# bcgsc/ntJoin

Hardware: AMD Instinct MI355X
Metric: Gbp/s minimizer-sketch+graph-build (k=32,w=1000) (higher is better)
Workload: dtype u64

## Files before the change

ntjoin_amd/csrc/graph.hip:

```cpp
#include <algorithm>
#include <cstdlib>
#include <cstring>
#include <system_error>
#include <thread>

#include "join_verdict.h"
#include "mxg_internal.h"
#include "scan_kernels.h"

namespace mxg {

static constexpr uint64_t HT_EMPTY = 0xFFFFFFFFFFFFFFFFull;
static constexpr uint32_t NONE32 = 0xFFFFFFFFu;

struct Slot {
    unsigned long long key;
    uint32_t nseen, ndup;
};

__device__ __forceinline__ uint32_t ht_slot(Slot *tab, uint32_t mask, uint32_t cap, uint64_t key)
{
    if (key == HT_EMPTY) return cap;
    uint32_t s = (uint32_t)((key * 0x9E3779B97F4A7C15ull) >> 32) & mask;
    while (true) {
// ... 158 lines not shown
            const uint32_t cb = hist[b0 + u];
            start[b0 + u] = run;
            row[b0 + u] = run;
            hist[b0 + u] = 0;
            run += cb;
        }
    if (threadIdx.x == 0) row[P] = sh[255];
    __syncthreads();
#pragma unroll
    for (uint32_t u = 0; u < U; ++u) {
        if (!((live >> u) & 1u)) continue;
        const uint32_t blk = blk0 + u * BPU + sub;
        uint32_t a = a0, i = ib0 + (u * BPU + sub) * 256u + t256;
        if (!one) {
            a = asm_of_block(p, blk);
            i = (blk - p.bstart[a]) * 256u + t256;
        }
        const uint32_t b = pj_part(key[u], pmask);
        const uint32_t pos = j * PJ_IPB + start[b] + atomicAdd(&hist[b], 1u);
        recs[pos] = make_uint4((uint32_t)key[u], (uint32_t)(key[u] >> 32), i, a | (((dupm >> u) & 1u) ? PJ_REC_DUP : 0u));
    }
}

__device__ __forceinline__ uint32_t pj_slot(unsigned long long *keys, uint64_t key)
{
    if (key == HT_EMPTY) return PJ_T;
    uint32_t s = (uint32_t)((key * 0x9E3779B97F4A7C15ull) >> 32) & (PJ_T - 1u);
    for (uint32_t step = 0; step < PJ_T; ++step) {
        const unsigned long long cur = keys[s];
        if (cur == key) return s;
        if (cur == HT_EMPTY) {
            const unsigned long long old = atomicCAS(&keys[s], (unsigned long long)HT_EMPTY, (unsigned long long)key);
            if (old == HT_EMPTY || old == key) return s;
        }
        s = (s + 1u) & (PJ_T - 1u);
    }
    return PJ_T + 1u;
}

struct PjSub {
    uint32_t n_sub, s, off, cap;
};
struct PjSubCaps {
    uint32_t n_sub;
    uint32_t cap[MXG_MAX_ASSEMBLIES];
};
template <bool NARROW>
__global__ __launch_bounds__(256) void k_pj_join(uint4 *recs, const uint32_t *__restrict__ M, uint32_t P, uint32_t n_rows,
                                                 uint64_t *host_fail, uint32_t force_fail, const uint32_t *__restrict__ cursor,
                                                 uint32_t cap1, uint32_t rows2, const AsmSet p, const PjSubCaps caps)
{
    const uint32_t full = p.full;
    __shared__ unsigned long long keys[PJ_T + 1];
    __shared__ uint32_t seen[PJ_T + 1], dup[NARROW ? 1 : PJ_T + 1];
    __shared__ uint32_t item0[PJ_T + 1];
    __shared__ uint32_t seg_off[257], seg_rec[256], sh[256];
    __shared__ uint32_t failed;
    uint32_t b = blockIdx.x, rec_off = 0;
    if (cursor) {
        const uint32_t c = blockIdx.x / P;
        b = blockIdx.x % P;
        n_rows = caps.n_sub > 1 ? rows2 : (min(cursor[c * PJ1_CS], cap1) + PJ_IPB - 1) / PJ_IPB;
        M += (size_t)c * rows2 * (P + 1);
        rec_off = c * cap1;
        if (threadIdx.x == 0)
            for (uint32_t s = 0; s < caps.n_sub; ++s)
                if (cursor[(c * caps.n_sub + s) * PJ1_CS] > caps.cap[s]) *host_fail = 1;
    }
    for (uint32_t s = threadIdx.x; s <= PJ_T; s += 256) {
        keys[s] = HT_EMPTY;
        seen[s] = 0;
        if (!NARROW) dup[s] = 0;
    }
// ... 42 lines not shown
                                if (NARROW) atomicOr(&seen[s], bit | (bit << 16));
                                else {
                                    atomicOr(&seen[s], bit);
                                    atomicOr(&dup[s], bit);
                                }
                            } else if (atomicOr(&seen[s], bit) & bit) {
                                if (NARROW) atomicOr(&seen[s], bit << 16); else atomicOr(&dup[s], bit);
                            }
                            if (last_a == 0) item0[s] = rec.z;
                        }
                    }
                }
                return s;
            };
            auto insert = [&](uint32_t r) { return insert_rec(recs[r]); };
            auto finish = [&](uint32_t i, uint32_t s, uint32_t a) {
                uint32_t fl = 0;
                if (!bad) {
                    const uint32_t sn = seen[s] & full, d = (NARROW ? seen[s] >> 16 : dup[s]) & full;
                    const bool inall = sn == full;
                    fl = (!(d & (1u << a)) ? MXG_MX_UNIQUE : 0u) | ((inall && d == 0) ? MXG_MX_SHARED : 0u) | (inall ? MXG_MX_INALL : 0u);
                }
                const uint32_t word = ((fl & MXG_MX_SHARED) ? item0[s] << 3 : 0u) | fl;
                if (!pj_verdict_is_prefill(word)) p.slot[a][i] = word;
            };
#pragma unroll
            for (uint32_t it = 0; it < QC; ++it) {
                const uint32_t q = threadIdx.x + it * 256u;
                if (q >= total) break;
                if (pass == 0) {
                    rc[it] = locate(q);
                    sc[it] = insert(rc[it]);
                    ac[it] = last_a;
                    ic[it] = last_i;
                } else if (single) {
                    finish(ic[it], sc[it], ac[it]);
                } else {
                    const uint32_t r = locate(q);
                    const uint32_t s = insert(r);
                    finish(last_i, s, last_a);
                }
            }
            constexpr uint32_t TU = 8;
            for (uint32_t q0 = threadIdx.x + QC * 256u; q0 < total; q0 += 256u * TU) {
                uint4 rv[TU];
#pragma unroll
                for (uint32_t u = 0; u < TU; ++u) {
                    const uint32_t q = q0 + u * 256u;
                    rv[u] = q < total ? recs[locate(q)] : make_uint4(0u, 0u, 0u, 0u);
                }
#pragma unroll
                for (uint32_t u = 0; u < TU; ++u) {
                    if (q0 + u * 256u >= total) break;
                    const uint32_t s = insert_rec(rv[u]);
                    if (pass == 1) finish(last_i, s, last_a);
                }
            }
            __syncthreads();
        }
    }
}


template <bool NARROW>
__global__ __launch_bounds__(256) void k_pj_join_pipe(uint4 *recs, const uint32_t *__restrict__ M, uint32_t P, uint32_t n_parts,
                                                      uint64_t *host_fail, uint32_t force_fail, const uint32_t *__restrict__ cursor,
                                                      uint32_t cap1, uint32_t rows2, const AsmSet p, const PjSubCaps caps)
{
    const uint32_t full = p.full;
    __shared__ unsigned long long keys[PJ_T + 1];
    __shared__ uint32_t seen[PJ_T + 1], dup[NARROW ? 1 : PJ_T + 1];
    __shared__ uint32_t item0[PJ_T + 1];
    __shared__ uint32_t seg_off[2][257], seg_rec[2][256], sh[256];
    __shared__ uint32_t failed;
    constexpr uint32_t QC = 4;
    __shared__ uint8_t seg_of[QC * 256];
    uint4 rn[QC];
    uint32_t tot_n = 0;
    uint32_t lo_nn = 0, len_nn = 0;
    auto bounds = [&](uint32_t part, uint32_t &lo, uint32_t &len) {
        lo = len = 0;
        if (part < n_parts && threadIdx.x < rows2) {
            const uint32_t c = part / P, b = part % P;
            const uint32_t *row = M + ((size_t)c * rows2 + threadIdx.x) * (P + 1);
            lo = row[b];
            len = row[b + 1];
        }
    };
    auto lay_out = [&](uint32_t part, uint32_t buf, uint32_t lo, uint32_t end) {
        const uint32_t c = part < n_parts ? part / P : 0u;
        const uint32_t len = end - lo;
        const uint32_t off = block_exclusive_256(len, sh);
        seg_off[buf][threadIdx.x] = off;
        seg_rec[buf][threadIdx.x] = c * cap1 + threadIdx.x * PJ_IPB + lo;
        for (uint32_t q = off, e = min(off + len, QC * 256u); q < e; ++q) seg_of[q] = (uint8_t)threadIdx.x;
        const uint32_t total = sh[255];
        __syncthreads();
#pragma unroll
        for (uint32_t it = 0; it < QC; ++it) {
            const uint32_t q = threadIdx.x + it * 256u;
            rn[it] = make_uint4(0u, 0u, 0u, 0u);
            if (q < total) {
                const uint32_t l = seg_of[q];
                rn[it] = recs[seg_rec[buf][l] + (q - seg_off[buf][l])];
            }
        }
        return total;
    };
    const uint32_t first = blockIdx.x, stride = gridDim.x;
    {
        uint32_t lo, end;
        bounds(first, lo, end);
        bounds(first + stride, lo_nn, len_nn);
        tot_n = lay_out(first, 0u, lo, end);
    }
    uint32_t k = 0;
    for (uint32_t part = first; part < n_parts; part += stride, ++k) {
        uint4 rc[QC];
#pragma unroll
        for (uint32_t it = 0; it < QC; ++it) rc[it] = rn[it];
        const uint32_t total = tot_n, buf = k & 1u;
        {
            const uint32_t lo = lo_nn, end = len_nn;
            bounds(part + 2u * stride, lo_nn, len_nn);
            tot_n = lay_out(part + stride, buf ^ 1u, lo, end);
        }
        for (uint32_t s = threadIdx.x; s <= PJ_T; s += 256) {
            keys[s] = HT_EMPTY;
            seen[s] = 0;
            if (!NARROW) dup[s] = 0;
        }
        if (threadIdx.x == 0) {
            failed = force_fail;
            const uint32_t c = part / P;
            if (part % P == 0)
                for (uint32_t s = 0; s < caps.n_sub; ++s)
                    if (cursor[(c * caps.n_sub + s) * PJ1_CS] > caps.cap[s]) *host_fail = 1;
        }
        __syncthreads();
        auto locate = [&](uint32_t q) {
            uint32_t l = 0, h = 256;
            while (h - l > 1) {
                const uint32_t m = (l + h) >> 1;
                if (seg_off[buf][m] <= q) l = m; else h = m;
            }
            return seg_rec[buf][l] + (q - seg_off[buf][l]);
        };
        auto insert_rec = [&](const uint4 rec, bool record) {
            const uint32_t a = rec.w & ~PJ_REC_DUP;
            const uint32_t s = pj_slot(keys, ((uint64_t)rec.y << 32) | rec.x);
            if (record) {
                const uint32_t bit = 1u << a;
                if (s > PJ_T) failed = 1;
                else {
                    const uint32_t cur = seen[s], dcur = NARROW ? cur >> 16 : dup[s];
                    if (!((cur & bit) && (dcur & bit))) {
                        if (rec.w & PJ_REC_DUP) {
                            if (NARROW) atomicOr(&seen[s], bit | (bit << 16));
                            else {
                                atomicOr(&seen[s], bit);
                                atomicOr(&dup[s], bit);
                            }
                        } else if (atomicOr(&seen[s], bit) & bit) {
                            if (NARROW) atomicOr(&seen[s], bit << 16); else atomicOr(&dup[s], bit);
                        }
                        if (a == 0) item0[s] = rec.z;
                    }
                }
            }
            return s;
        };
        uint32_t sc[QC];
#pragma unroll
        for (uint32_t it = 0; it < QC; ++it)
            if (threadIdx.x + it * 256u < total) sc[it] = insert_rec(rc[it], true);
        constexpr uint32_t TU = 8;
        for (uint32_t q0 = threadIdx.x + QC * 256u; q0 < total; q0 += 256u * TU) {
            uint4 rv[TU];
#pragma unroll
            for (uint32_t u = 0; u < TU; ++u) {
                const uint32_t q = q0 + u * 256u;
                rv[u] = q < total ? recs[locate(q)] : make_uint4(0u, 0u, 0u, 0u);
            }
#pragma unroll
            for (uint32_t u = 0; u < TU; ++u)
                if (q0 + u * 256u < total) insert_rec(rv[u], true);
        }
        __syncthreads();
        const bool bad = failed != 0;
        if (bad && threadIdx.x == 0) *host_fail = 1;
        auto finish = [&](const uint4 rec, uint32_t s) {
            const uint32_t a = rec.w & ~PJ_REC_DUP;
            uint32_t fl = 0;
            if (!bad) {
                const uint32_t sn = seen[s] & full, d = (NARROW ? seen[s] >> 16 : dup[s]) & full;
                const bool inall = sn == full;
                fl = (!(d & (1u << a)) ? MXG_MX_UNIQUE : 0u) | ((inall && d == 0) ? MXG_MX_SHARED : 0u) | (inall ? MXG_MX_INALL : 0u);
            }
            const uint32_t word = ((fl & MXG_MX_SHARED) ? item0[s] << 3 : 0u) | fl;
            if (!pj_verdict_is_prefill(word)) p.slot[a][rec.z] = word;
        };
#pragma unroll
        for (uint32_t it = 0; it < QC; ++it)
            if (threadIdx.x + it * 256u < total) finish(rc[it], bad ? 0u : sc[it]);
        for (uint32_t q0 = threadIdx.x + QC * 256u; q0 < total; q0 += 256u * TU) {
            uint4 rv[TU];
#pragma unroll
            for (uint32_t u = 0; u < TU; ++u) {
                const uint32_t q = q0 + u * 256u;
                rv[u] = q < total ? recs[locate(q)] : make_uint4(0u, 0u, 0u, 0u);
            }
#pragma unroll
            for (uint32_t u = 0; u < TU; ++u)
                if (q0 + u * 256u < total) finish(rv[u], bad ? 0u : insert_rec(rv[u], false));
        }
        __syncthreads();
    }
}

__device__ __forceinline__ uint32_t pj1_part(uint64_t key, uint32_t p1mask) { return (uint32_t)((key * 0x9E3779B97F4A7C15ull) >> 52) & p1mask; }

__global__ __launch_bounds__(PJ_BT) void k_pj1_scatter(const AsmSet p, uint32_t blk_lo, uint32_t blk_hi, uint32_t p1mask, uint32_t cap1,
                                                     uint32_t *cursor, uint4 *recs1, uint32_t *sup, uint32_t n_sup, const PjSub subr)
{
    extern __shared__ uint32_t pj_lds[];
    uint32_t *hist = pj_lds, *start = pj_lds + p1mask + 1;
    if (blockIdx.x == 0)
        for (uint32_t i = threadIdx.x; i < n_sup; i += PJ_BT) sup[i] = 0;
    constexpr uint32_t U = PJ_IPB / PJ_BT, BPU = PJ_BT / 256;
    const uint32_t j = blockIdx.x, sub = threadIdx.x >> 8, t256 = threadIdx.x & 255u;
    const uint32_t blk0 = blk_lo + j * (PJ_IPB / 256);
    uint64_t key[U];
    uint32_t ia[U], ii[U], live = 0;
#pragma unroll
    for (uint32_t u = 0; u < U; ++u) {
        const uint32_t blk = blk0 + u * BPU + sub;
        key[u] = 0;
        ia[u] = ii[u] = 0;
        if (blk >= blk_hi) continue;
        const uint32_t a = subr.n_sub > 1 ? subr.s : asm_of_block(p, blk);
        const uint32_t i = (blk - p.bstart[a]) * 256u + t256, n = asm_n(p, a);
        const bool lv = i < n;
        if (lv) {
            key[u] = p.hash[a][i];
            p.slot[a][i] = PJ_VERDICT_PREFILL;
        }
        const uint32_t role = pj_run_role(i, n, key[u], lv);
        const uint64_t fb = __ballot(role & 1u);
        if ((threadIdx.x & 63u) == 0) p.fol[(size_t)blk * 4u + ((threadIdx.x >> 6) & 3u)] = fb;
        if (lv && !(role & 1u)) {
            ia[u] = a | ((role & 2u) ? PJ_REC_DUP : 0u);
            ii[u] = i;
            live |= 1u << u;
        }
    }
    for (uint32_t b = threadIdx.x; b <= p1mask; b += PJ_BT) hist[b] = 0;
    __syncthreads();
#pragma unroll
    for (uint32_t u = 0; u < U; ++u)
        if ((live >> u) & 1u) atomicAdd(&hist[pj1_part(key[u], p1mask)], 1u);
    __syncthreads();
    for (uint32_t b = threadIdx.x; b <= p1mask; b += PJ_BT) {
        const uint32_t c = hist[b];
        start[b] = c ? atomicAdd(&cursor[(b * subr.n_sub + subr.s) * PJ1_CS], c) : 0u;
        hist[b] = 0;
    }
    __syncthreads();
#pragma unroll
    for (uint32_t u = 0; u < U; ++u) {
        if (!((live >> u) & 1u)) continue;
        const uint32_t b = pj1_part(key[u], p1mask);
        const uint32_t pos = start[b] + atomicAdd(&hist[b], 1u);
        if (pos < subr.cap) recs1[(size_t)b * cap1 + subr.off + pos] = make_uint4((uint32_t)key[u], (uint32_t)(key[u] >> 32), ii[u], ia[u]);
        else p.slot[ia[u] & ~PJ_REC_DUP][ii[u]] = 0;
    }
}

__global__ __launch_bounds__(PJ_BT) void k_pj2_bucket(const AsmSet p, const uint4 *__restrict__ recs1, const uint32_t *__restrict__ cursor,
                                                    uint32_t cap1, uint32_t rows2, uint32_t pmask, uint32_t *M, uint4 *recs2,
                                                    uint32_t skew_lim, const PjSub subr)
{
    extern __shared__ uint32_t pj_lds[];
    uint32_t *hist = pj_lds, *start = pj_lds + pmask + 1;
    __shared__ uint32_t sh[256];
    const uint32_t j = blockIdx.x, c = blockIdx.y;
    const uint32_t n_all = cursor[(c * subr.n_sub + subr.s) * PJ1_CS], n_c = min(n_all, subr.cap);
    const uint32_t row_j = subr.off / PJ_IPB + j;
    if (j * PJ_IPB >= n_c) {
        uint32_t *row = M + ((size_t)c * rows2 + row_j) * (pmask + 2);
        for (uint32_t b = threadIdx.x; b <= pmask + 1; b += PJ_BT) row[b] = 0;
        return;
    }
    constexpr uint32_t U = PJ_IPB / PJ_BT;
    const size_t base = (size_t)c * cap1 + subr.off + (size_t)j * PJ_IPB;
    uint4 rec[U];
    uint32_t live = 0;
#pragma unroll
    for (uint32_t u = 0; u < U; ++u) {
        const uint32_t q = u * PJ_BT + threadIdx.x;
        rec[u] = make_uint4(0u, 0u, 0u, 0u);
        if (j * PJ_IPB + q < n_c) {
            rec[u] = recs1[base + q];
            live |= 1u << u;
        }
    }
    if (n_all > skew_lim) {
        __shared__ unsigned long long skey[PJ_IPB];
        __shared__ uint32_t sitem[PJ_IPB];
        __shared__ uint8_t sasm[PJ_IPB];
        __shared__ uint32_t stab[PJ_IPB];
        __shared__ uint32_t sdup[PJ_IPB / 32];
        for (uint32_t q = threadIdx.x; q < PJ_IPB; q += PJ_BT) stab[q] = 0xFFFFFFFFu;
        for (uint32_t q = threadIdx.x; q < PJ_IPB / 32; q += PJ_BT) sdup[q] = 0;
#pragma unroll
        for (uint32_t u = 0; u < U; ++u) {
            const uint32_t q = u * PJ_BT + threadIdx.x;
            skey[q] = ((unsigned long long)rec[u].y << 32) | rec[u].x;
            sitem[q] = rec[u].z;
            sasm[q] = (uint8_t)(rec[u].w & 0xFFu);
        }
        __syncthreads();
#pragma unroll
        for (uint32_t u = 0; u < U; ++u) {
            if (!((live >> u) & 1u)) continue;
            const uint32_t q = u * PJ_BT + threadIdx.x;
// ... 12 lines not shown
                if (skey[cur] == key && sasm[cur] == a) {
                    rep = cur;
                    break;
                }
                hsl = (hsl + 1u) & (2u * PJ_IPB - 1u);
            }
            if (rep != q) {
                atomicOr(&sdup[rep >> 5], 1u << (rep & 31u));
                p.slot[a][rec[u].z] = (sitem[rep] << 3) | PJ_VERDICT_REF;
                live &= ~(1u << u);
            }
        }
        __syncthreads();
#pragma unroll
        for (uint32_t u = 0; u < U; ++u) {
            const uint32_t q = u * PJ_BT + threadIdx.x;
            if ((sdup[q >> 5] >> (q & 31u)) & 1u) rec[u].w |= PJ_REC_DUP;
        }
    }
    for (uint32_t b = threadIdx.x; b <= pmask; b += PJ_BT) hist[b] = 0;
    __syncthreads();
#pragma unroll
    for (uint32_t u = 0; u < U; ++u)
        if ((live >> u) & 1u) atomicAdd(&hist[pj_part(((uint64_t)rec[u].y << 32) | rec[u].x, pmask)], 1u);
    __syncthreads();
    const uint32_t P = pmask + 1, per = P >= PJ_BT ? P / PJ_BT : 1u, b0 = threadIdx.x * per;
    uint32_t cn = 0;
    if (b0 < P)
        for (uint32_t u = 0; u < per; ++u) cn += hist[b0 + u];
    uint32_t run = block_exclusive<PJ_BT / 64>(cn, sh);
    uint32_t *row = M + ((size_t)c * rows2 + row_j) * (P + 1);
    if (b0 < P)
        for (uint32_t u = 0; u < per; ++u) {
            const uint32_t cb = hist[b0 + u];
            start[b0 + u] = run;
            row[b0 + u] = run;
            hist[b0 + u] = 0;
            run += cb;
        }
    if (threadIdx.x == 0) row[P] = sh[255];
    __syncthreads();
#pragma unroll
    for (uint32_t u = 0; u < U; ++u) {
        if (!((live >> u) & 1u)) continue;
        const uint32_t b = pj_part(((uint64_t)rec[u].y << 32) | rec[u].x, pmask);
        const uint32_t pos = (uint32_t)base + start[b] + atomicAdd(&hist[b], 1u);
        recs2[pos] = rec[u];
    }
}

template <uint32_t U>
struct TailScan {
    uint32_t tot[U][4];
    uint32_t before[U];
};
template <uint32_t U>
__device__ __forceinline__ void tail_ballot(TailScan<U> &ts, uint32_t u, bool f, uint64_t &bm)
{
    bm = __ballot(f);
    if ((threadIdx.x & 63u) == 0) ts.tot[u][threadIdx.x >> 6] = (uint32_t)__popcll(bm);
}
template <uint32_t U>
__device__ __forceinline__ uint32_t tail_rank(const TailScan<U> &ts, uint32_t u, uint64_t bm)
{
    const uint32_t lane = threadIdx.x & 63u, wv = threadIdx.x >> 6;
    uint32_t r = (uint32_t)__popcll(bm & ((1ull << lane) - 1ull));
#pragma unroll
    for (uint32_t q = 0; q < 3; ++q) r += q < wv ? ts.tot[u][q] : 0u;
    return r;
}
// ... 501 lines not shown
};

static int plan_join(mxg_handle *h, int mode, const GraphBounds *gb, bool global_table, bool split, JoinPlan &pl)
{
    const uint32_t A = (uint32_t)h->asms.size();
    if (A == 0) return set_err(h, MXG_EINVAL, "mxg_build_graph: no assemblies");
    if (A > MXG_MAX_ASSEMBLIES) return set_err(h, MXG_ELIMIT, "at most %d assemblies", MXG_MAX_ASSEMBLIES);
    pl = JoinPlan();
    JoinRequest rq;
    rq.A = A;
    for (uint32_t ai = 0; ai < A; ++ai) {
        Assembly *a = h->asms[ai];
        if (!gb && !a->has_sketch) return set_err(h, MXG_EINVAL, "assembly '%s' has no sketch (call mxg_sketch)", a->name.c_str());
        rq.n_of[ai] = gb ? gb->n_bound[ai] : a->n_mx;
    }
    rq.mode = mode;
    rq.bounds = gb != nullptr;
    rq.global_table = global_table;
    rq.split = split;
    const char *join_env = knob_raw(h, "MXG_GRAPH_JOIN");
    rq.join_global = join_env && !strcmp(join_env, "global");
    rq.force_two_level = knob_u64(h, "MXG_PJ_TWO_LEVEL", 0) != 0;
    rq.graph_u = (uint32_t)std::min<uint64_t>(knob_u64(h, "MXG_GRAPH_U", 0), 8);
    switch (join_shape(rq, h->pj_learnt, pl)) {
    case JS_TOO_MANY_MINIMIZERS: return set_err(h, MXG_ELIMIT, "too many minimizers for one table (%llu)", (unsigned long long)pl.N);
    case JS_TOO_MANY_ITEMS: return set_err(h, MXG_ELIMIT, "graph too large for 32-bit item indices");
    case JS_OK: break;
    }
    pl.pj_force_fail = knob_u64(h, "MXG_PJ_FORCE_FAIL", 0) ? 1u : 0u;
    pl.sc.n_sub = pl.n_sub;
    for (uint32_t a = 0; a < MXG_MAX_ASSEMBLIES; ++a) pl.sc.cap[a] = pl.sub_cap[a];
    const uint64_t *const n_of = pl.n_of;
    const uint32_t nb = pl.nb, P = pl.P, P1 = pl.P1;

    if (!pl.pj) MXG_HIP(h, h->g_keys.ensure(((size_t)pl.cap + 1) * sizeof(Slot)));
    const size_t nb0 = pl.nb0, nb_all = nb;
    MXG_HIP(h, h->g_vid.ensure(pl.pj ? (nb0 + nb_all) * 4 * 8 + nb0 * 4 + 64 : ((size_t)pl.cap + 1) * 4));
    pl.pj_mask0 = h->g_vid.as<uint64_t>();
    uint64_t *const pj_fol = pl.pj_mask0 + nb0 * 4;
    pl.pj_bpref0 = reinterpret_cast<uint32_t *>(pj_fol + nb_all * 4);
    MXG_HIP(h, h->g_ctl.ensure(CTL_WORDS * 8));

    AsmSet &as_all = pl.as_all;
    as_all.n_asm = A;
    as_all.full = pl.full;
    as_all.fol = pl.pj ? pj_fol : nullptr;
// ... 27 lines not shown
        const size_t n_recs = (size_t)P1 * pl.cap1;
        MXG_HIP(h, h->g_part.ensure((size_t)P1 * pl.rows2 * (P + 1) * 4 + (size_t)P1 * PJ1_CS * 4));
        MXG_HIP(h, h->g_keys.ensure(n_recs * sizeof(uint4)));
        MXG_HIP(h, h->g_recs1.ensure(n_recs * sizeof(uint4)));
        pl.M = h->g_part.as<uint32_t>();
        pl.cursor = pl.n_cur ? pl.esup + pl.n_esup : pl.M + (size_t)P1 * pl.rows2 * (P + 1);
        pl.recs1 = h->g_recs1.as<uint4>();
        pl.recs2 = h->g_keys.as<uint4>();
    }
    return MXG_OK;
}

static void launch_partition(mxg_handle *h, const JoinPlan &pl, uint32_t a_lo, uint32_t a_hi, hipStream_t st, uint32_t n_sup_clear)
{
    const uint32_t blk_lo = pl.as_all.bstart[a_lo], blk_hi = pl.as_all.bstart[a_hi];
    const uint32_t n_rows1 = (blk_hi - blk_lo + PJ_IPB / 256 - 1) / (PJ_IPB / 256);
    PjSub sub{1u, 0u, 0u, pl.cap1};
    uint32_t skew_lim = (uint32_t)std::min<uint64_t>(pl.N / pl.P1 + pl.N / pl.P1 / 32 + 2048, 0xFFFFFFFFull);
    if (pl.split) {
        sub = PjSub{pl.A, a_lo, pl.sub_off[a_lo], pl.sub_cap[a_lo]};
        skew_lim = pl.skew_lim[a_lo];
    }
    if (n_rows1)
        hipLaunchKernelGGL(k_pj1_scatter, dim3(n_rows1), dim3(PJ_BT), (size_t)pl.P1 * 8, st, pl.as_all, blk_lo, blk_hi, pl.P1 - 1, pl.cap1,
                           pl.cursor, pl.recs1, pl.fsup, n_sup_clear, sub);
    hipLaunchKernelGGL(k_pj2_bucket, dim3(sub.cap / PJ_IPB, pl.P1), dim3(PJ_BT), (size_t)pl.P * 8, st, pl.as_all, pl.recs1, pl.cursor, pl.cap1,
                       pl.rows2, pl.P - 1, pl.M, pl.recs2, knob_u64(h, "MXG_PJ_SKEW", 0) ? 0u : skew_lim, sub);
}

static int ev_pair(mxg_handle *h, hipEvent_t *a, hipEvent_t *b)
{
    while (h->ev_pool.size() < h->ev_used + 2) {
        hipEvent_t e;
        MXG_HIP(h, hipEventCreate(&e));
        h->ev_pool.push_back(e);
    }
    *a = h->ev_pool[h->ev_used];
    *b = h->ev_pool[h->ev_used + 1];
    h->ev_used += 2;
    h->ev_spans.push_back(TimedSpan{*a, *b, 0, false, 5});
    return MXG_OK;
}

int graph_plan_early(mxg_handle *h, const GraphBounds &gb, bool *early)
{
    *early = false;
    h->pj_early_done = 0;
    if (knob_u64(h, "MXG_PJ_EARLY", 1) == 0) return MXG_OK;
    MXG_HIP(h, hipSetDevice(h->device));
    if (!h->pj_plan) h->pj_plan = new JoinPlan;
// ... 75 lines not shown
          fine((h_->cfg.flags & MXG_FLAG_TIMING_FINE) != 0 && c_.mode == GRAPH_FULL), timing((h_->cfg.flags & MXG_FLAG_TIMING) != 0 || fine),
          g(h_->graph)
    {
    }
    bool joins() const { return pl.nb && !resume; }
    size_t anv() const { return (size_t)pl.A * pl.nvs; }

    int begin()
    {
        for (uint32_t ai = 0; ai < pl.A; ++ai) {
            Assembly *a = h->asms[ai];
            if (!resume) a->flags_on_host = false;
            a->flags_valid = true;
        }
        if (!resume) g = Graph();
        g.n_asm = pl.A;
        if (fine && !h->ev_g[0]) {
            MXG_HIP(h, hipEventCreate(&h->ev_g[0]));
            MXG_HIP(h, hipEventCreate(&h->ev_g[1]));
        }
        if (timing) MXG_HIP(h, hipEventRecord(h->ev0, h->stream));
        if (!resume)
            h->stat_graph_join = (pl.pj ? (pl.two_level ? MXG_JOIN_LDS_TWO_LEVEL : MXG_JOIN_LDS) : MXG_JOIN_GLOBAL) | (early ? MXG_JOIN_EARLY : 0);
        if (!pl.pj && !resume) MXG_HIP(h, hipMemsetAsync(h->g_keys.p, 0xFF, ((size_t)pl.cap + 1) * sizeof(Slot), h->stream));
        ctl = h->g_ctl.as<uint64_t>();
        if (!h->pinned_gctl) MXG_HIP(h, hipHostMalloc((void **)&h->pinned_gctl, CTL_WORDS * 8));
        hctl = h->pinned_gctl;
        memset(hctl, 0, CTL_WORDS * 8);
        pj_fail = pl.dg_pj ? dg_pj_fail_word(h) : hctl + CTL_PJ_FAIL;
        return MXG_OK;
    }

    void launch_join(uint4 *recs, uint32_t *M, uint32_t n_parts, uint32_t n_rows, const uint32_t *cursor)
    {
        const bool narrow = pl.A <= 16;
        const uint32_t cap1 = cursor ? pl.cap1 : 0u, rows2 = cursor ? pl.rows2 : 0u;
        const uint64_t pipe_blocks = cursor ? knob_u64(h, "MXG_PJ_PIPE", 1024) : 0;
        if (pipe_blocks && rows2 <= 256)
            hipLaunchKernelGGL(narrow ? k_pj_join_pipe<true> : k_pj_join_pipe<false>, dim3((uint32_t)std::min<uint64_t>(pipe_blocks, n_parts)),
                               dim3(256), 0, h->stream, recs, M, pl.P, n_parts, pj_fail, pl.pj_force_fail, cursor, cap1, rows2, pl.as_all, pl.sc);
        else
            hipLaunchKernelGGL(narrow ? k_pj_join<true> : k_pj_join<false>, dim3(n_parts), dim3(256), 0, h->stream, recs, M, pl.P, n_rows,
                               pj_fail, pl.pj_force_fail, cursor, cap1, rows2, pl.as_all, pl.sc);
    }
    void flags_pj()
    {
        TAIL_LAUNCH(k_flags_pj, pl.u_flags, dim3(graph_tail_grid(pl.nb, pl.u_flags)), h->stream, pl.as_all, pl.nb, pl.cnt, pl.fsup, pl.pj_mask0);
    }
    int join_two_level()
    {
        if (!early) {
            MXG_HIP(h, hipMemsetAsync(pl.cursor, 0, (size_t)pl.P1 * PJ1_CS * 4, h->stream));
            launch_partition(h, pl, 0, pl.A, h->stream, pl.n_fsup + pl.n_esup);
        }
        launch_join(pl.recs2, pl.M, pl.P1 * pl.P, 0u, pl.cursor);
        flags_pj();
        return MXG_OK;
    }
    int join_one_level()
    {
        const uint32_t n_rows = (pl.nb + PJ_IPB / 256 - 1) / (PJ_IPB / 256);
        MXG_HIP(h, h->g_part.ensure((size_t)n_rows * (pl.P + 1) * 4));
        MXG_HIP(h, h->g_keys.ensure((size_t)n_rows * PJ_IPB * sizeof(uint4)));
        uint32_t *M = h->g_part.as<uint32_t>();
        uint4 *recs = h->g_keys.as<uint4>();
        hipLaunchKernelGGL(k_pj_bucket, dim3(n_rows), dim3(PJ_BT), (size_t)pl.P * 8, h->stream, pl.as_all, pl.nb, pl.P - 1, M, recs, pl.fsup,
                           pl.n_fsup + pl.n_esup);
        launch_join(recs, M, pl.P, n_rows, nullptr);
        flags_pj();
        return MXG_OK;
    }
    int join_global()
    {
        hipLaunchKernelGGL(k_insert, dim3(pl.nb), dim3(256), 0, h->stream, pl.as_all, h->g_keys.as<Slot>(), pl.mask, pl.cap, pl.fsup,
// ... 151 lines not shown
        TAIL_LAUNCH(k_edges, pl.u_edges, grid, h->stream, ep, n_items);
        MXG_HIP(h, hipGetLastError());
        return MXG_OK;
    }

    int sync_and_verdict()
    {
        if (timing) MXG_HIP(h, hipEventRecord(h->ev1, h->stream));
        MXG_HIP(h, stream_wait(h->stream));
        if (!pl.pj || !hctl[CTL_PJ_FAIL]) return MXG_OK;
        if (!pl.two_level || pl.pj_force_fail) return RC_RETRY_GLOBAL;
        std::vector<uint32_t> cur((size_t)pl.P1 * pl.n_sub * PJ1_CS);
        MXG_HIP(h, hipMemcpy(cur.data(), pl.cursor, cur.size() * 4, hipMemcpyDeviceToHost));
        return join_overflow_verdict(pl, cur.data(), h->pj_learnt);
    }
    int results()
    {
        const uint64_t nv = hctl[CTL_SHARED];
        for (uint32_t a = 1; a < pl.A; ++a)
            if (hctl[CTL_SHARED + a] != nv)
                return set_err(h, MXG_EDEVICE, "internal error: shared-minimizer counts differ between assemblies (%llu vs %llu)",
                               (unsigned long long)hctl[CTL_SHARED + a], (unsigned long long)nv);
        g.nv = nv;
        g.nv_stride = pl.nvs;
        g.ne = pl.nvs > 0 ? hctl[CTL_EDGES] : 0;
        h->stat_unique = ~0ull;
        if (timing) {
            float ms = 0;
            MXG_HIP(h, hipEventElapsedTime(&ms, h->ev0, h->ev1));
            h->tm.ms_graph += ms;
            if (fine && pl.nvs > 0) {
                float a = 0, b = 0, c3 = 0;
                MXG_HIP(h, hipEventElapsedTime(&a, h->ev0, h->ev_g[0]));
                MXG_HIP(h, hipEventElapsedTime(&b, h->ev_g[0], h->ev_g[1]));
                MXG_HIP(h, hipEventElapsedTime(&c3, h->ev_g[1], h->ev1));
                h->tm.ms_join += a;
                h->tm.ms_vertices += b;
                h->tm.ms_edges += c3;
            }
        }
        g.valid = true;
        g.own_order = c.mode == GRAPH_FULL;
        g.host_valid = false;
        return MXG_OK;
    }
};
// ... 88 lines not shown
```

ntjoin_amd/csrc/join_plan.h:

```cpp
#pragma once
#include <algorithm>
#include <cstddef>
#include <cstdint>

#include "ntjoin_mx.h"

namespace mxg {

enum { GRAPH_FULL = 0, GRAPH_DG_VERTICES = 1, GRAPH_DG_EDGES = 2, GRAPH_DG_EDGES_APPLIED = 3  };

constexpr uint32_t PJ_IPB = 4096;
constexpr uint32_t PJ_T = 2048;
constexpr uint32_t PJ_MAX_P = 4096;
constexpr uint32_t PJ1_CS = 32;
constexpr uint32_t PJ_CAP_LIMIT = 0xFFFFF000u;

struct JoinLearnt {
    bool overflowed = false;
    uint32_t cap1_P1 = 0;
    uint64_t cap1_need = 0;
    uint64_t sig = 0;
    uint32_t sub_P1 = 0;
    uint64_t sub_need[MXG_MAX_ASSEMBLIES] = {};
    bool dg_off = false;

    static uint64_t signature(uint32_t n_asm, const uint64_t *n_mx)
    {
        uint64_t s = 0x9E3779B97F4A7C15ull * ((uint64_t)n_asm + 1);
        for (uint32_t a = 0; a < n_asm; ++a) s = (s ^ n_mx[a]) * 0x100000001B3ull;
        return s;
    }
    void sketches_are(uint64_t s)
    {
        if ((overflowed || cap1_P1) && sig != s) {
            overflowed = false;
            cap1_P1 = 0;
            cap1_need = 0;
            sub_P1 = 0;
        }
        sig = s;
    }
    void assembly_added()
    {
        overflowed = false;
        cap1_P1 = 0;
        cap1_need = 0;
    }
    void gave_up() { overflowed = true; }
};

struct JoinRequest {
    uint32_t A = 0;
    uint64_t n_of[MXG_MAX_ASSEMBLIES] = {};
    int mode = GRAPH_FULL;
    bool bounds = false;
    bool global_table = false;
    bool split = false;
    bool force_two_level = false;
    bool join_global = false;
    uint32_t graph_u = 0;
};

enum JoinShapeError { JS_OK = 0, JS_TOO_MANY_MINIMIZERS, JS_TOO_MANY_ITEMS };

struct JoinShape {
    uint32_t A = 0;
    uint64_t N = 0, nvs = 0;
    uint64_t n_of[MXG_MAX_ASSEMBLIES] = {};
    uint32_t cap = 0, mask = 0, full = 0;
    uint32_t P = 0, P1 = 0, cap1 = 0, rows2 = 0;
    bool two_level = false, pj = false, dg_pj = false;
    bool split = false;
    uint32_t n_sub = 1;
    uint32_t sub_cap[MXG_MAX_ASSEMBLIES] = {}, sub_off[MXG_MAX_ASSEMBLIES] = {}, skew_lim[MXG_MAX_ASSEMBLIES] = {};
    uint32_t bstart[MXG_MAX_ASSEMBLIES + 1] = {};
    uint32_t nb = 0;
    size_t nb0 = 0;
    uint32_t n_items = 0, e_blocks = 0;
    size_t n_cur = 0;
    uint32_t u_flags = 1, u_vertices = 1, u_edges = 1;
};

constexpr uint32_t GRAPH_TAIL_U2 = 3072, GRAPH_TAIL_U4 = 8192;
constexpr uint32_t GRAPH_TAIL_U_VERTICES = 2;
inline uint32_t graph_tail_u(uint64_t blocks, uint32_t forced = 0)
{
    if (forced == 1 || forced == 2 || forced == 4) return forced;
    return blocks >= GRAPH_TAIL_U4 ? 4u : blocks >= GRAPH_TAIL_U2 ? 2u : 1u;
}
inline uint32_t graph_tail_grid(uint64_t blocks, uint32_t U) { return (uint32_t)((blocks + U - 1) / U); }

inline JoinShapeError join_shape(const JoinRequest &rq, const JoinLearnt &learnt, JoinShape &pl)
{
    pl = JoinShape();
    const uint32_t A = pl.A = rq.A;
    uint64_t N = 0, nmin = ~0ull, n_max = 0;
    for (uint32_t a = 0; a < A; ++a) {
        pl.n_of[a] = rq.n_of[a];
        N += rq.n_of[a];
        nmin = std::min(nmin, rq.n_of[a]);
        n_max = std::max(n_max, rq.n_of[a]);
// ... 34 lines not shown
            cap1 = (uint32_t)((c1 + PJ_IPB - 1) / PJ_IPB * PJ_IPB);
            pl.sub_cap[0] = cap1;
        }
        pl.rows2 = cap1 / PJ_IPB;
    }
    pl.P = P;
    pl.P1 = P1;
    pl.cap1 = cap1;
    pl.two_level = P1 != 0 && P1 <= 4096 && fits32 && (uint64_t)P1 * cap1 < (1ull << 32) && (uint64_t)P1 * P * (PJ_T + 1) < (1ull << 29);
    pl.dg_pj = rq.mode == GRAPH_DG_VERTICES && rq.bounds && !learnt.dg_off;
    pl.pj = (rq.mode == GRAPH_FULL || pl.dg_pj) && !rq.global_table && (P1 == 0 || pl.two_level) && P <= PJ_MAX_P && n_max < (1ull << 29) &&
            !rq.join_global;
    for (uint32_t a = 0; a < A; ++a) {
        pl.bstart[a] = pl.nb;
        pl.nb += (uint32_t)((rq.n_of[a] + 255) / 256);
    }
    for (uint32_t a = A; a <= MXG_MAX_ASSEMBLIES; ++a) pl.bstart[a] = pl.nb;
    pl.nb0 = (size_t)((rq.n_of[0] + 255) / 256);
    pl.nvs = nmin;
    if (pl.nvs > 0 && (uint64_t)A * pl.nvs >= (1ull << 32)) return JS_TOO_MANY_ITEMS;
    pl.n_items = (uint32_t)((size_t)A * pl.nvs);
    pl.e_blocks = (pl.n_items + 255) / 256;
    if (pl.split && pl.pj && pl.two_level) pl.n_cur = (size_t)P1 * A * PJ1_CS;
    pl.u_flags = graph_tail_u(pl.nb, rq.graph_u);
    pl.u_vertices = graph_tail_u(0, rq.graph_u) == rq.graph_u ? rq.graph_u : std::min(pl.u_flags, GRAPH_TAIL_U_VERTICES);
    pl.u_edges = graph_tail_u(pl.e_blocks, rq.graph_u);
    return JS_OK;
}

enum JoinRetry { RC_RETRY_GLOBAL = 1, RC_RETRY_PJ = 2 };

inline JoinRetry join_overflow_verdict(const JoinShape &pl, const uint32_t *cur, JoinLearnt &learnt)
{
    const uint32_t P1 = pl.P1, n_sub = pl.n_sub;
    uint64_t mx = 0;
    for (uint32_t c = 0; c < P1; ++c) {
        uint64_t all = 0;
        for (uint32_t s = 0; s < n_sub; ++s) all += cur[((size_t)c * n_sub + s) * PJ1_CS];
        mx = std::max(mx, all);
    }
    if (pl.split) {
        bool grew = false;
        if (learnt.sub_P1 != P1) std::fill_n(learnt.sub_need, MXG_MAX_ASSEMBLIES, 0ull);
        learnt.sub_P1 = P1;
        for (uint32_t s = 0; s < n_sub; ++s) {
            uint64_t ms = 0;
// ... 22 lines not shown
```

ntjoin_amd/csrc/join_verdict.h:

```cpp
#pragma once
#include <cstdint>

#include "ntjoin_mx.h"

#if defined(__HIPCC__)
#define PJV_HD __host__ __device__ inline
#else
#define PJV_HD inline
#endif

namespace mxg {

constexpr uint32_t PJ_VERDICT_PREFILL = MXG_MX_UNIQUE;
constexpr uint32_t PJ_VERDICT_REF = 2u;

PJV_HD bool pj_verdict_is_prefill(uint32_t word) { return word == PJ_VERDICT_PREFILL; }

}
```

Measured before the change: 2709.

## Pack join records to 12 bytes and learn a shared-prefill verdict

Join records shrink from 16 to 12 bytes. The assembly tag and dup flag are folded into key bits that the partition index already implies, and keys are pre-multiplied so the partition and slot come straight from the stored bits. A learnt prefill rule writes the likely shared verdict for assembly 0 up front so fewer verdict stores are needed on later runs. It also adds a split-per-assembly partition path and debug knobs, which makes the bit-packing and learnt state more complex and adds correctness risk.

```diff
diff --git a/ntjoin_amd/csrc/graph.hip b/ntjoin_amd/csrc/graph.hip
--- a/ntjoin_amd/csrc/graph.hip
+++ b/ntjoin_amd/csrc/graph.hip
@@ -204,10 +204,9 @@
     }
 }
 
-__device__ __forceinline__ uint32_t pj_slot(unsigned long long *keys, uint64_t key)
+__device__ __forceinline__ uint32_t pj_slot_from(unsigned long long *keys, uint64_t key, uint32_t s)
 {
     if (key == HT_EMPTY) return PJ_T;
-    uint32_t s = (uint32_t)((key * 0x9E3779B97F4A7C15ull) >> 32) & (PJ_T - 1u);
     for (uint32_t step = 0; step < PJ_T; ++step) {
         const unsigned long long cur = keys[s];
         if (cur == key) return s;
@@ -218,6 +217,27 @@
         s = (s + 1u) & (PJ_T - 1u);
     }
     return PJ_T + 1u;
+}
+__device__ __forceinline__ uint32_t pj_slot(unsigned long long *keys, uint64_t key)
+{
+    return pj_slot_from(keys, key, (uint32_t)((key * 0x9E3779B97F4A7C15ull) >> 32) & (PJ_T - 1u));
+}
+
+struct PjRec3 {
+    uint32_t x, y, z;
+};
+template <bool R12>
+__device__ __forceinline__ uint4 pj_rec_load(const uint4 *recs, size_t r)
+{
+    if (!R12) return recs[r];
+    const PjRec3 v = reinterpret_cast<const PjRec3 *>(recs)[r];
+    return make_uint4(v.x, v.y, v.z, 0u);
+}
+template <bool R12>
+__device__ __forceinline__ void pj_rec_store(uint4 *recs, size_t r, const uint4 v)
+{
+    if (!R12) recs[r] = v;
+    else reinterpret_cast<PjRec3 *>(recs)[r] = PjRec3{v.x, v.y, v.z};
 }
 
 struct PjSub {
@@ -230,7 +250,7 @@
 template <bool NARROW>
 __global__ __launch_bounds__(256) void k_pj_join(uint4 *recs, const uint32_t *__restrict__ M, uint32_t P, uint32_t n_rows,
                                                  uint64_t *host_fail, uint32_t force_fail, const uint32_t *__restrict__ cursor,
-                                                 uint32_t cap1, uint32_t rows2, const AsmSet p, const PjSubCaps caps)
+                                                 uint32_t cap1, uint32_t rows2, const AsmSet p, const PjSubCaps caps, uint32_t prefill0)
 {
     const uint32_t full = p.full;
     __shared__ unsigned long long keys[PJ_T + 1];
@@ -319,7 +339,7 @@
                     fl = (!(d & (1u << a)) ? MXG_MX_UNIQUE : 0u) | ((inall && d == 0) ? MXG_MX_SHARED : 0u) | (inall ? MXG_MX_INALL : 0u);
                 }
                 const uint32_t word = ((fl & MXG_MX_SHARED) ? item0[s] << 3 : 0u) | fl;
-                if (!pj_verdict_is_prefill(word)) p.slot[a][i] = word;
+                if (word != pj_verdict_prefill(prefill0, a, i)) p.slot[a][i] = word;
             };
 #pragma unroll
             for (uint32_t it = 0; it < QC; ++it) {
@@ -359,12 +379,19 @@
 }
 
 
-template <bool NARROW>
+template <bool NARROW, bool R12>
 __global__ __launch_bounds__(256) void k_pj_join_pipe(uint4 *recs, const uint32_t *__restrict__ M, uint32_t P, uint32_t n_parts,
                                                       uint64_t *host_fail, uint32_t force_fail, const uint32_t *__restrict__ cursor,
-                                                      uint32_t cap1, uint32_t rows2, const AsmSet p, const PjSubCaps caps)
+                                                      uint32_t cap1, uint32_t rows2, const AsmSet p, const PjSubCaps caps, uint32_t prefill0)
 {
     const uint32_t full = p.full;
+    const uint32_t lgP = R12 ? 31u - (uint32_t)__clz(P) : 0u, tag_mask = R12 ? pj12_tag_mask(lgP) : 0u;
+    auto rec_a = [&](const uint4 rec) { return R12 ? pj12_unpack_tag(rec.y, lgP) & (PJ12_TAG_DUP - 1u) : rec.w & ~PJ_REC_DUP; };
+    auto rec_dup = [&](const uint4 rec) { return R12 ? (pj12_unpack_tag(rec.y, lgP) & PJ12_TAG_DUP) != 0 : (rec.w & PJ_REC_DUP) != 0; };
+    auto rec_slot = [&](unsigned long long *tab, const uint4 rec) {
+        if (R12) return pj_slot_from(tab, ((uint64_t)(rec.y & ~tag_mask) << 32) | rec.x, rec.y & (PJ_T - 1u));
+        return pj_slot(tab, ((uint64_t)rec.y << 32) | rec.x);
+    };
     __shared__ unsigned long long keys[PJ_T + 1];
     __shared__ uint32_t seen[PJ_T + 1], dup[NARROW ? 1 : PJ_T + 1];
     __shared__ uint32_t item0[PJ_T + 1];
@@ -399,7 +426,7 @@
             rn[it] = make_uint4(0u, 0u, 0u, 0u);
             if (q < total) {
                 const uint32_t l = seg_of[q];
-                rn[it] = recs[seg_rec[buf][l] + (q - seg_off[buf][l])];
+                rn[it] = pj_rec_load<R12>(recs, seg_rec[buf][l] + (q - seg_off[buf][l]));
             }
         }
         return total;
@@ -444,15 +471,15 @@
             return seg_rec[buf][l] + (q - seg_off[buf][l]);
         };
         auto insert_rec = [&](const uint4 rec, bool record) {
-            const uint32_t a = rec.w & ~PJ_REC_DUP;
-            const uint32_t s = pj_slot(keys, ((uint64_t)rec.y << 32) | rec.x);
+            const uint32_t a = rec_a(rec);
+            const uint32_t s = rec_slot(keys, rec);
             if (record) {
                 const uint32_t bit = 1u << a;
                 if (s > PJ_T) failed = 1;
                 else {
                     const uint32_t cur = seen[s], dcur = NARROW ? cur >> 16 : dup[s];
                     if (!((cur & bit) && (dcur & bit))) {
-                        if (rec.w & PJ_REC_DUP) {
+                        if (rec_dup(rec)) {
                             if (NARROW) atomicOr(&seen[s], bit | (bit << 16));
                             else {
                                 atomicOr(&seen[s], bit);
@@ -477,7 +504,7 @@
 #pragma unroll
             for (uint32_t u = 0; u < TU; ++u) {
                 const uint32_t q = q0 + u * 256u;
-                rv[u] = q < total ? recs[locate(q)] : make_uint4(0u, 0u, 0u, 0u);
+                rv[u] = q < total ? pj_rec_load<R12>(recs, locate(q)) : make_uint4(0u, 0u, 0u, 0u);
             }
 #pragma unroll
             for (uint32_t u = 0; u < TU; ++u)
@@ -487,7 +514,7 @@
         const bool bad = failed != 0;
         if (bad && threadIdx.x == 0) *host_fail = 1;
         auto finish = [&](const uint4 rec, uint32_t s) {
-            const uint32_t a = rec.w & ~PJ_REC_DUP;
+            const uint32_t a = rec_a(rec);
             uint32_t fl = 0;
             if (!bad) {
                 const uint32_t sn = seen[s] & full, d = (NARROW ? seen[s] >> 16 : dup[s]) & full;
@@ -495,7 +522,7 @@
                 fl = (!(d & (1u << a)) ? MXG_MX_UNIQUE : 0u) | ((inall && d == 0) ? MXG_MX_SHARED : 0u) | (inall ? MXG_MX_INALL : 0u);
             }
             const uint32_t word = ((fl & MXG_MX_SHARED) ? item0[s] << 3 : 0u) | fl;
-            if (!pj_verdict_is_prefill(word)) p.slot[a][rec.z] = word;
+            if (word != pj_verdict_prefill(prefill0, a, rec.z)) p.slot[a][rec.z] = word;
         };
 #pragma unroll
         for (uint32_t it = 0; it < QC; ++it)
@@ -505,7 +532,7 @@
 #pragma unroll
             for (uint32_t u = 0; u < TU; ++u) {
                 const uint32_t q = q0 + u * 256u;
-                rv[u] = q < total ? recs[locate(q)] : make_uint4(0u, 0u, 0u, 0u);
+                rv[u] = q < total ? pj_rec_load<R12>(recs, locate(q)) : make_uint4(0u, 0u, 0u, 0u);
             }
 #pragma unroll
             for (uint32_t u = 0; u < TU; ++u)
@@ -517,9 +544,12 @@
 
 __device__ __forceinline__ uint32_t pj1_part(uint64_t key, uint32_t p1mask) { return (uint32_t)((key * 0x9E3779B97F4A7C15ull) >> 52) & p1mask; }
 
+template <bool R12>
 __global__ __launch_bounds__(PJ_BT) void k_pj1_scatter(const AsmSet p, uint32_t blk_lo, uint32_t blk_hi, uint32_t p1mask, uint32_t cap1,
-                                                     uint32_t *cursor, uint4 *recs1, uint32_t *sup, uint32_t n_sup, const PjSub subr)
-{
+                                                     uint32_t *cursor, uint4 *recs1, uint32_t *sup, uint32_t n_sup, const PjSub subr,
+                                                     uint32_t prefill0)
+{
+    auto part1 = [&](uint64_t k) { return R12 ? (uint32_t)(k >> 52) & p1mask : pj1_part(k, p1mask); };
     extern __shared__ uint32_t pj_lds[];
     uint32_t *hist = pj_lds, *start = pj_lds + p1mask + 1;
     if (blockIdx.x == 0)
@@ -540,11 +570,12 @@
         const bool lv = i < n;
         if (lv) {
             key[u] = p.hash[a][i];
-            p.slot[a][i] = PJ_VERDICT_PREFILL;
+            p.slot[a][i] = pj_verdict_prefill(prefill0, a, i);
         }
         const uint32_t role = pj_run_role(i, n, key[u], lv);
         const uint64_t fb = __ballot(role & 1u);
         if ((threadIdx.x & 63u) == 0) p.fol[(size_t)blk * 4u + ((threadIdx.x >> 6) & 3u)] = fb;
+        if (R12) key[u] *= PJ_MUL;
         if (lv && !(role & 1u)) {
             ia[u] = a | ((role & 2u) ? PJ_REC_DUP : 0u);
             ii[u] = i;
@@ -555,7 +586,7 @@
     __syncthreads();
 #pragma unroll
     for (uint32_t u = 0; u < U; ++u)
-        if ((live >> u) & 1u) atomicAdd(&hist[pj1_part(key[u], p1mask)], 1u);
+        if ((live >> u) & 1u) atomicAdd(&hist[part1(key[u])], 1u);
     __syncthreads();
     for (uint32_t b = threadIdx.x; b <= p1mask; b += PJ_BT) {
         const uint32_t c = hist[b];
@@ -566,13 +597,16 @@
 #pragma unroll
     for (uint32_t u = 0; u < U; ++u) {
         if (!((live >> u) & 1u)) continue;
-        const uint32_t b = pj1_part(key[u], p1mask);
+        const uint32_t b = part1(key[u]);
         const uint32_t pos = start[b] + atomicAdd(&hist[b], 1u);
-        if (pos < subr.cap) recs1[(size_t)b * cap1 + subr.off + pos] = make_uint4((uint32_t)key[u], (uint32_t)(key[u] >> 32), ii[u], ia[u]);
+        if (pos < subr.cap)
+            pj_rec_store<R12>(recs1, (size_t)b * cap1 + subr.off + pos,
+                              make_uint4((uint32_t)key[u], (uint32_t)(key[u] >> 32), R12 && (ia[u] & PJ_REC_DUP) ? ii[u] | PJ12_ITEM_DUP : ii[u], ia[u]));
         else p.slot[ia[u] & ~PJ_REC_DUP][ii[u]] = 0;
     }
 }
 
+template <bool R12>
 __global__ __launch_bounds__(PJ_BT) void k_pj2_bucket(const AsmSet p, const uint4 *__restrict__ recs1, const uint32_t *__restrict__ cursor,
                                                     uint32_t cap1, uint32_t rows2, uint32_t pmask, uint32_t *M, uint4 *recs2,
                                                     uint32_t skew_lim, const PjSub subr)
@@ -581,6 +615,8 @@
     uint32_t *hist = pj_lds, *start = pj_lds + pmask + 1;
     __shared__ uint32_t sh[256];
     const uint32_t j = blockIdx.x, c = blockIdx.y;
+    const uint32_t lgP = R12 ? 31u - (uint32_t)__clz(pmask + 1u) : 0u;
+    auto part2 = [&](const uint4 r) { return R12 ? (r.y >> PJ12_FINE_SHIFT) & pmask : pj_part(((uint64_t)r.y << 32) | r.x, pmask); };
     const uint32_t n_all = cursor[(c * subr.n_sub + subr.s) * PJ1_CS], n_c = min(n_all, subr.cap);
     const uint32_t row_j = subr.off / PJ_IPB + j;
     if (j * PJ_IPB >= n_c) {
@@ -597,7 +633,11 @@
         const uint32_t q = u * PJ_BT + threadIdx.x;
         rec[u] = make_uint4(0u, 0u, 0u, 0u);
         if (j * PJ_IPB + q < n_c) {
-            rec[u] = recs1[base + q];
+            rec[u] = pj_rec_load<R12>(recs1, base + q);
+            if (R12) {
+                rec[u].w = subr.s | ((rec[u].z & PJ12_ITEM_DUP) ? PJ_REC_DUP : 0u);
+                rec[u].z &= ~PJ12_ITEM_DUP;
+            }
             live |= 1u << u;
         }
     }
@@ -656,7 +696,7 @@
     __syncthreads();
 #pragma unroll
     for (uint32_t u = 0; u < U; ++u)
-        if ((live >> u) & 1u) atomicAdd(&hist[pj_part(((uint64_t)rec[u].y << 32) | rec[u].x, pmask)], 1u);
+        if ((live >> u) & 1u) atomicAdd(&hist[part2(rec[u])], 1u);
     __syncthreads();
     const uint32_t P = pmask + 1, per = P >= PJ_BT ? P / PJ_BT : 1u, b0 = threadIdx.x * per;
     uint32_t cn = 0;
@@ -677,9 +717,10 @@
 #pragma unroll
     for (uint32_t u = 0; u < U; ++u) {
         if (!((live >> u) & 1u)) continue;
-        const uint32_t b = pj_part(((uint64_t)rec[u].y << 32) | rec[u].x, pmask);
+        const uint32_t b = part2(rec[u]);
         const uint32_t pos = (uint32_t)base + start[b] + atomicAdd(&hist[b], 1u);
-        recs2[pos] = rec[u];
+        if (R12) rec[u].y = pj12_pack(rec[u].y, lgP, pj12_tag(rec[u].w & ~PJ_REC_DUP, (rec[u].w & PJ_REC_DUP) != 0));
+        pj_rec_store<R12>(recs2, pos, rec[u]);
     }
 }
 
@@ -1227,6 +1268,10 @@
     rq.join_global = join_env && !strcmp(join_env, "global");
     rq.force_two_level = knob_u64(h, "MXG_PJ_TWO_LEVEL", 0) != 0;
     rq.graph_u = (uint32_t)std::min<uint64_t>(knob_u64(h, "MXG_GRAPH_U", 0), 8);
+    rq.no_rec12 = knob_u64(h, "MXG_PJ_REC12", 1) == 0;
+    rq.no_pipe = knob_u64(h, "MXG_PJ_PIPE", 1024) == 0;
+    rq.no_prefill0 = knob_u64(h, "MXG_PJ_PREFILL0", 1) == 0;
+    if (knob_u64(h, "MXG_PJ_SPLIT", 0) && mode == GRAPH_FULL) rq.split = true;
     switch (join_shape(rq, h->pj_learnt, pl)) {
     case JS_TOO_MANY_MINIMIZERS: return set_err(h, MXG_ELIMIT, "too many minimizers for one table (%llu)", (unsigned long long)pl.N);
     case JS_TOO_MANY_ITEMS: return set_err(h, MXG_ELIMIT, "graph too large for 32-bit item indices");
@@ -1300,10 +1345,11 @@
         skew_lim = pl.skew_lim[a_lo];
     }
     if (n_rows1)
-        hipLaunchKernelGGL(k_pj1_scatter, dim3(n_rows1), dim3(PJ_BT), (size_t)pl.P1 * 8, st, pl.as_all, blk_lo, blk_hi, pl.P1 - 1, pl.cap1,
-                           pl.cursor, pl.recs1, pl.fsup, n_sup_clear, sub);
-    hipLaunchKernelGGL(k_pj2_bucket, dim3(sub.cap / PJ_IPB, pl.P1), dim3(PJ_BT), (size_t)pl.P * 8, st, pl.as_all, pl.recs1, pl.cursor, pl.cap1,
-                       pl.rows2, pl.P - 1, pl.M, pl.recs2, knob_u64(h, "MXG_PJ_SKEW", 0) ? 0u : skew_lim, sub);
+        hipLaunchKernelGGL(pl.rec12 ? k_pj1_scatter<true> : k_pj1_scatter<false>, dim3(n_rows1), dim3(PJ_BT), (size_t)pl.P1 * 8, st, pl.as_all,
+                           blk_lo, blk_hi, pl.P1 - 1, pl.cap1, pl.cursor, pl.recs1, pl.fsup, n_sup_clear, sub, pl.prefill0);
+    hipLaunchKernelGGL(pl.rec12 ? k_pj2_bucket<true> : k_pj2_bucket<false>, dim3(sub.cap / PJ_IPB, pl.P1), dim3(PJ_BT), (size_t)pl.P * 8, st,
+                       pl.as_all, pl.recs1, pl.cursor, pl.cap1, pl.rows2, pl.P - 1, pl.M, pl.recs2,
+                       knob_u64(h, "MXG_PJ_SKEW", 0) ? 0u : skew_lim, sub);
 }
 
 static int ev_pair(mxg_handle *h, hipEvent_t *a, hipEvent_t *b)
@@ -1425,6 +1471,9 @@
         if (timing) MXG_HIP(h, hipEventRecord(h->ev0, h->stream));
         if (!resume)
             h->stat_graph_join = (pl.pj ? (pl.two_level ? MXG_JOIN_LDS_TWO_LEVEL : MXG_JOIN_LDS) : MXG_JOIN_GLOBAL) | (early ? MXG_JOIN_EARLY : 0);
+        if (!resume && knob_u64(h, "MXG_DEBUG_JOIN", 0))
+            fprintf(stderr, "[mxg] join pj=%d two_level=%d split=%d early=%d record_bytes=%d prefill0=%u P1=%u rows2=%u\n", (int)pl.pj,
+                    (int)pl.two_level, (int)pl.split, (int)early, pl.rec12 ? 12 : 16, pl.prefill0, pl.P1, pl.rows2);
         if (!pl.pj && !resume) MXG_HIP(h, hipMemsetAsync(h->g_keys.p, 0xFF, ((size_t)pl.cap + 1) * sizeof(Slot), h->stream));
         ctl = h->g_ctl.as<uint64_t>();
         if (!h->pinned_gctl) MXG_HIP(h, hipHostMalloc((void **)&h->pinned_gctl, CTL_WORDS * 8));
@@ -1439,12 +1488,15 @@
         const bool narrow = pl.A <= 16;
         const uint32_t cap1 = cursor ? pl.cap1 : 0u, rows2 = cursor ? pl.rows2 : 0u;
         const uint64_t pipe_blocks = cursor ? knob_u64(h, "MXG_PJ_PIPE", 1024) : 0;
-        if (pipe_blocks && rows2 <= 256)
-            hipLaunchKernelGGL(narrow ? k_pj_join_pipe<true> : k_pj_join_pipe<false>, dim3((uint32_t)std::min<uint64_t>(pipe_blocks, n_parts)),
-                               dim3(256), 0, h->stream, recs, M, pl.P, n_parts, pj_fail, pl.pj_force_fail, cursor, cap1, rows2, pl.as_all, pl.sc);
-        else
+        const uint32_t prefill0 = cursor ? pl.prefill0 : 0u;
+        if (pipe_blocks && rows2 <= 256) {
+            auto kernel = pl.rec12 ? (narrow ? k_pj_join_pipe<true, true> : k_pj_join_pipe<false, true>)
+                                   : (narrow ? k_pj_join_pipe<true, false> : k_pj_join_pipe<false, false>);
+            hipLaunchKernelGGL(kernel, dim3((uint32_t)std::min<uint64_t>(pipe_blocks, n_parts)), dim3(256), 0, h->stream, recs, M, pl.P, n_parts,
+                               pj_fail, pl.pj_force_fail, cursor, cap1, rows2, pl.as_all, pl.sc, prefill0);
+        } else
             hipLaunchKernelGGL(narrow ? k_pj_join<true> : k_pj_join<false>, dim3(n_parts), dim3(256), 0, h->stream, recs, M, pl.P, n_rows,
-                               pj_fail, pl.pj_force_fail, cursor, cap1, rows2, pl.as_all, pl.sc);
+                               pj_fail, pl.pj_force_fail, cursor, cap1, rows2, pl.as_all, pl.sc, prefill0);
     }
     void flags_pj()
     {
@@ -1452,7 +1504,10 @@
     }
     int join_two_level()
     {
-        if (!early) {
+        if (!early && pl.split) {
+            MXG_HIP(h, hipMemsetAsync(pl.fsup, 0, pl.clear_words * 4, h->stream));
+            for (uint32_t a = 0; a < pl.A; ++a) launch_partition(h, pl, a, a + 1, h->stream, 0u);
+        } else if (!early) {
             MXG_HIP(h, hipMemsetAsync(pl.cursor, 0, (size_t)pl.P1 * PJ1_CS * 4, h->stream));
             launch_partition(h, pl, 0, pl.A, h->stream, pl.n_fsup + pl.n_esup);
         }
@@ -1650,6 +1705,7 @@
                 return set_err(h, MXG_EDEVICE, "internal error: shared-minimizer counts differ between assemblies (%llu vs %llu)",
                                (unsigned long long)hctl[CTL_SHARED + a], (unsigned long long)nv);
         g.nv = nv;
+        if (c.mode == GRAPH_FULL) h->pj_learnt.shared_counted(pl.pre_sig, nv, pl.n_of[0]);
         g.nv_stride = pl.nvs;
         g.ne = pl.nvs > 0 ? hctl[CTL_EDGES] : 0;
         h->stat_unique = ~0ull;
diff --git a/ntjoin_amd/csrc/join_plan.h b/ntjoin_amd/csrc/join_plan.h
--- a/ntjoin_amd/csrc/join_plan.h
+++ b/ntjoin_amd/csrc/join_plan.h
@@ -4,6 +4,12 @@
 #include <cstdint>
 
 #include "ntjoin_mx.h"
+
+#if defined(__HIPCC__)
+#define PJP_HD __host__ __device__ inline
+#else
+#define PJP_HD inline
+#endif
 
 namespace mxg {
 
@@ -23,6 +29,8 @@
     uint32_t sub_P1 = 0;
     uint64_t sub_need[MXG_MAX_ASSEMBLIES] = {};
     bool dg_off = false;
+    bool pre_known = false;
+    uint64_t pre_sig = 0, pre_shared0 = 0, pre_n0 = 0;
 
     static uint64_t signature(uint32_t n_asm, const uint64_t *n_mx)
     {
@@ -42,12 +50,62 @@
     }
     void assembly_added()
     {
+        pre_known = false;
         overflowed = false;
         cap1_P1 = 0;
         cap1_need = 0;
     }
     void gave_up() { overflowed = true; }
+
+    static uint64_t prefill_signature(uint32_t n_asm, const uint64_t *n_of, bool bounds)
+    {
+        return signature(n_asm, n_of) ^ (bounds ? 0xB0B0B0B0B0B0B0B0ull : 0ull);
+    }
+    void shared_counted(uint64_t plan_sig, uint64_t shared0, uint64_t n0)
+    {
+        pre_known = true;
+        pre_sig = plan_sig;
+        pre_shared0 = shared0;
+        pre_n0 = n0;
+    }
+    bool prefill_own0(uint64_t plan_sig) const { return pre_known && pre_sig == plan_sig && 2 * pre_shared0 > pre_n0; }
 };
+
+constexpr uint64_t PJ_MUL = 0x9E3779B97F4A7C15ull;
+constexpr uint32_t PJ12_TAG_BITS = 6, PJ12_TAG_DUP = 32u, PJ12_ITEM_DUP = 0x80000000u;
+constexpr uint32_t PJ12_FINE_SHIFT = 44 - 32, PJ12_COARSE_SHIFT = 52 - 32;
+
+PJP_HD uint32_t pj12_lg(uint32_t x)
+{
+    uint32_t n = 0;
+    while ((1u << n) < x && n < 31) ++n;
+    return n;
+}
+PJP_HD bool pj12_fits(uint32_t P1, uint32_t P) { return P1 != 0 && P != 0 && (uint64_t)P1 * P >= (1u << PJ12_TAG_BITS); }
+PJP_HD uint32_t pj12_fine_bits(uint32_t lgP) { return lgP < PJ12_TAG_BITS ? lgP : PJ12_TAG_BITS; }
+PJP_HD uint32_t pj12_tag_mask(uint32_t lgP)
+{
+    const uint32_t f = pj12_fine_bits(lgP);
+    return (((1u << f) - 1u) << PJ12_FINE_SHIFT) | (((1u << (PJ12_TAG_BITS - f)) - 1u) << PJ12_COARSE_SHIFT);
+}
+PJP_HD uint32_t pj12_tag(uint32_t assembly, bool dup) { return assembly | (dup ? PJ12_TAG_DUP : 0u); }
+PJP_HD uint32_t pj12_pack(uint32_t prod_hi, uint32_t lgP, uint32_t tag)
+{
+    const uint32_t f = pj12_fine_bits(lgP);
+    return (prod_hi & ~pj12_tag_mask(lgP)) | ((tag & ((1u << f) - 1u)) << PJ12_FINE_SHIFT) | ((tag >> f) << PJ12_COARSE_SHIFT);
+}
+PJP_HD uint32_t pj12_unpack_tag(uint32_t word, uint32_t lgP)
+{
+    const uint32_t f = pj12_fine_bits(lgP);
+    return ((word >> PJ12_FINE_SHIFT) & ((1u << f) - 1u)) | (((word >> PJ12_COARSE_SHIFT) & ((1u << (PJ12_TAG_BITS - f)) - 1u)) << f);
+}
+PJP_HD uint64_t pj12_key(uint32_t lo, uint32_t word, uint32_t lgP) { return ((uint64_t)(word & ~pj12_tag_mask(lgP)) << 32) | lo; }
+PJP_HD bool pj12_same_key(uint32_t lo_a, uint32_t word_a, uint32_t lo_b, uint32_t word_b, uint32_t lgP)
+{
+    return pj12_key(lo_a, word_a, lgP) == pj12_key(lo_b, word_b, lgP);
+}
+PJP_HD uint32_t pj12_coarse(uint64_t prod, uint32_t P1) { return (uint32_t)(prod >> 52) & (P1 - 1u); }
+PJP_HD uint32_t pj12_fine(uint64_t prod, uint32_t P) { return (uint32_t)(prod >> 44) & (P - 1u); }
 
 struct JoinRequest {
     uint32_t A = 0;
@@ -58,6 +116,9 @@
     bool split = false;
     bool force_two_level = false;
     bool join_global = false;
+    bool no_rec12 = false;
+    bool no_pipe = false;
+    bool no_prefill0 = false;
     uint32_t graph_u = 0;
 };
 
@@ -77,6 +138,9 @@
     uint32_t nb = 0;
     size_t nb0 = 0;
     uint32_t n_items = 0, e_blocks = 0;
+    bool rec12 = false;
+    uint32_t prefill0 = 0;
+    uint64_t pre_sig = 0;
     size_t n_cur = 0;
     uint32_t u_flags = 1, u_vertices = 1, u_edges = 1;
 };
@@ -157,6 +221,9 @@
     pl.n_items = (uint32_t)((size_t)A * pl.nvs);
     pl.e_blocks = (pl.n_items + 255) / 256;
     if (pl.split && pl.pj && pl.two_level) pl.n_cur = (size_t)P1 * A * PJ1_CS;
+    pl.rec12 = pl.split && pl.pj && pl.two_level && pj12_fits(P1, P) && pl.rows2 <= 256 && !rq.no_rec12 && !rq.no_pipe;
+    pl.pre_sig = JoinLearnt::prefill_signature(A, rq.n_of, rq.bounds);
+    pl.prefill0 = pl.pj && pl.two_level && !rq.no_prefill0 && learnt.prefill_own0(pl.pre_sig) ? 1u : 0u;
     pl.u_flags = graph_tail_u(pl.nb, rq.graph_u);
     pl.u_vertices = graph_tail_u(0, rq.graph_u) == rq.graph_u ? rq.graph_u : std::min(pl.u_flags, GRAPH_TAIL_U_VERTICES);
     pl.u_edges = graph_tail_u(pl.e_blocks, rq.graph_u);
diff --git a/ntjoin_amd/csrc/join_verdict.h b/ntjoin_amd/csrc/join_verdict.h
--- a/ntjoin_amd/csrc/join_verdict.h
+++ b/ntjoin_amd/csrc/join_verdict.h
@@ -16,4 +16,12 @@
 
 PJV_HD bool pj_verdict_is_prefill(uint32_t word) { return word == PJ_VERDICT_PREFILL; }
 
+enum PjPrefillRule : uint32_t { PJ_PREFILL_UNIQUE = 0, PJ_PREFILL_OWN0 = 1 };
+constexpr uint32_t PJ_VERDICT_SHARED = MXG_MX_UNIQUE | MXG_MX_SHARED | MXG_MX_INALL;
+
+PJV_HD uint32_t pj_verdict_prefill(uint32_t rule, uint32_t a, uint32_t i)
+{
+    return rule == PJ_PREFILL_OWN0 && a == 0 ? (i << 3) | PJ_VERDICT_SHARED : PJ_VERDICT_PREFILL;
 }
+
+}
```

Result: faster. 2757 (median of 6 runs) (+1.8%).
